# leggedrobotics/elevation_mapping_cupy

Hardware: NVIDIA B200
Metric: Mpoints/s fused + map-update frames/s (1024^2 grid, 200k-pt LiDAR frames, raycast+overlap-clear on) (higher is better)
Workload: dtype f32

## Files before the change

elevation_mapping_cupy_b200/csrc/emap_api.cu:

```cuda
#include <cmath>
#include <cstdio>
#include <cstdlib>
#include <cstring>
#include <mutex>
#include <string>
#include <vector>

#include <dlfcn.h>
#include <nvtx3/nvToolsExt.h>

#include "../../include/emap.h"
#include "emap_kernels.cuh"
#include "emap_inpaint.cuh"
#include "emap_semantic.cuh"

namespace {

thread_local std::string g_create_error;

struct StageTimer {
  cudaEvent_t ev[9];
  bool have = false;
};

// ... 292 lines not shown
      o += bytes;
    }
    CK(cudaEventRecord(h->copy_done, h->copy_stream));
    CK(cudaStreamWaitEvent(h->stream, h->copy_done, 0));
  }
  h->pend_pts.assign(dp, dp + n_sensors);
  h->pend_n.assign(n, n + n_sensors);
  h->pend_stride = row_stride; h->pend_dtype = dtype; h->pend_host = !is_device_ptr;
  h->phase = -1;
  return 0;
}

int frame_index(emap_handle* h) {
  NvtxRange nv("emap:index+error");
  const int n_sensors = (int)h->pend_pts.size();
  for (int s = 0; s < n_sensors; s++) {
    int rc = h->pend_dtype == EMAP_F32
                 ? launch_index<float>(h, h->poses[s], (const float*)h->pend_pts[s], h->pend_n[s], h->pend_stride, h->offs[s], s)
                 : launch_index<double>(h, h->poses[s], (const double*)h->pend_pts[s], h->pend_n[s], h->pend_stride, h->offs[s], s);
    if (rc) return rc;
  }
  if (h->pend_host) CK(cudaEventRecord(h->in_free[h->in_sel ^ 1], h->stream));
  if (h->zero_copy_pending) CK(cudaEventRecord(h->copy_done, h->stream));
  if (stage_mark(h, 1)) return EMAP_ERR_CUDA;
  h->phase = 1;
  return 0;
}

int frame_fuse(emap_handle* h) {
  NvtxRange nv("emap:drift+fusion");
  const float overlap_tz = h->overlap_override ? h->overlap_z_override : h->poses[0].t[2];
  if (!h->fused_drift) {
    PDL(k_drift, 1, 256, 0, h->dc, h->fs, h->pos_noise, h->ori_noise, overlap_tz, 1, h->tmap);
    LAUNCH_CHECK();
  }
  if (stage_mark(h, 2)) return EMAP_ERR_CUDA;
  if (h->fused_drift) {
    PDL((k_fuse<3, 1>), std::max(1, cdiv(h->n_points, 256)), 256, 0, h->dc, h->n_points, h->global_off, (const float4*)h->xyzv,
        (const int*)h->pidx, (const float*)h->map, h->sc, (const FrameScalars*)h->fs, h->fs, h->pos_noise, h->ori_noise, overlap_tz);
    LAUNCH_CHECK();
  } else if (h->n_points > 0) {
    if (h->attached) {
      PDL((k_fuse<1, 0>), cdiv(h->n_points, 256), 256, 0, h->dc, h->n_points, h->global_off, (const float4*)h->xyzv,
          (const int*)h->pidx, (const float*)h->map, h->sc, (const FrameScalars*)h->fs, h->fs, 0.f, 0.f, 0.f);
    } else {
      PDL((k_fuse<3, 0>), cdiv(h->n_points, 256), 256, 0, h->dc, h->n_points, h->global_off, (const float4*)h->xyzv,
          (const int*)h->pidx, (const float*)h->map, h->sc, (const FrameScalars*)h->fs, h->fs, 0.f, 0.f, 0.f);
    }
    LAUNCH_CHECK();
  }
  if (stage_mark(h, 3)) return EMAP_ERR_CUDA;
  h->phase = 2;
  return 0;
}

template <typename T>
int launch_sem_sum(emap_handle* h, const T* pts, i64 n, i64 stride, i64 off) {
  if (n <= 0) return 0;
  k_sem_sum<T><<<cdiv(n, 256), 256, 0, h->stream>>>(h->dc, h->sem, pts, n, stride, (const int*)(h->pidx + off), h->sem_fsum, h->sem_csum);
  LAUNCH_CHECK();
  return 0;
}

int frame_semantic(emap_handle* h) {
  if (h->sem.n_ch <= 0 || !h->sem_map) return 0;
  NvtxRange nv("emap:semantic");
  for (size_t s = 0; s < h->pend_pts.size(); s++) {
    int rc = h->pend_dtype == EMAP_F32
                 ? launch_sem_sum<float>(h, (const float*)h->pend_pts[s], h->pend_n[s], h->pend_stride, h->offs[s])
                 : launch_sem_sum<double>(h, (const double*)h->pend_pts[s], h->pend_n[s], h->pend_stride, h->offs[s]);
    if (rc) return rc;
  }
  if (h->pend_host) CK(cudaEventRecord(h->in_free[h->in_sel ^ 1], h->stream));
  if (h->zero_copy_pending) CK(cudaEventRecord(h->copy_done, h->stream));
  k_sem_apply<<<cdiv(h->dc.C, 256), 256, 0, h->stream>>>(h->dc, h->sem, (const u64*)h->sc.cnt_fo, h->sem_fsum, h->sem_csum, h->sem_map);
  LAUNCH_CHECK();
  return 0;
}

RayGrid ray_grid(const emap_handle* h, int align) {
  const int W = h->dc.W;
  int r0 = W, r1 = 0, c0 = W, c1 = 0;
  const double L = (double)h->dc.max_len16;
  for (const Pose& q : h->poses) {
    for (int ax = 0; ax < 2; ax++) {
      const double tc = (double)q.t[ax];
      const double e = (std::fabs(tc) + L) * (1.0 / 2048.0) + 1e-4;
      double lo = std::floor((tc - L - e) / h->dc.resolution + h->dc.half_w) - 2.0;
      double hi = std::floor((tc + L + e) / h->dc.resolution + h->dc.half_w) + 3.0;
      if (!(lo == lo) || !(hi == hi)) { lo = 0; hi = W; }
      const int a = (int)std::min(std::max(lo, 0.0), (double)W), b = (int)std::min(std::max(hi, 0.0), (double)W);
      if (ax == 0) { r0 = std::min(r0, a); r1 = std::max(r1, b); } else { c0 = std::min(c0, a); c1 = std::max(c1, b); }
    }
  }
  RayGrid g{0, 0, 0, 0, 3, 0, 0};
  if (r1 <= r0 || c1 <= c0) return g;
  c0 = (c0 / align) * align; c1 = std::min(W, ((c1 + align - 1) / align) * align);
  g.r0 = r0; g.r1 = r1; g.c0 = c0; g.c1 = c1;
  for (int ts = 2;; ts++) {
    const int al = 2 << ts;
    const int r0a = (r0 / al) * al, c0a = (c0 / al) * al;
    if ((RT << ts) >= std::max(r1 - r0a, c1 - c0a) && (4 << ts) >= h->span_cells + 1) {
      g.ts = ts; g.ta = r0a >> ts; g.tb = c0a >> ts;
      break;
    }
  }
  return g;
}

int frame_rays(emap_handle* h) {
  NvtxRange nv("emap:record+raycast");
  const bool deferred = h->attached && h->n_points > 0;
  if (deferred) {
    CK(cudaEventRecord(h->ev_fork, h->stream));
    CK(cudaStreamWaitEvent(h->side_stream, h->ev_fork, 0));
    k_fuse<2, 0><<<cdiv(h->n_points, 256), 256, 0, h->side_stream>>>(h->dc, h->n_points, h->global_off, (const float4*)h->xyzv,
                                                                       (const int*)h->pidx, (const float*)h->map, h->sc,
                                                                       (const FrameScalars*)h->fs, h->fs, 0.f, 0.f, 0.f);
    LAUNCH_CHECK();
    CK(cudaEventRecord(h->ev_join, h->side_stream));
  }
  if (h->dc.visibility) {
    const int V = (h->dc.W % 4 == 0) ? 4 : 1;
    const RayGrid box = ray_grid(h, V);
    const i64 nthreads = (i64)(box.r1 - box.r0) * ((box.c1 - box.c0) / V);
    if (nthreads > 0) {
      if (V == 4) PDL(k_record<4>, cdiv(nthreads, 256), 256, 0, h->dc, (const float*)h->map, h->sc, (const FrameScalars*)h->fs, box, h->tmap);
      else PDL(k_record<1>, cdiv(nthreads, 256), 256, 0, h->dc, (const float*)h->map, h->sc, (const FrameScalars*)h->fs, box, h->tmap);
      LAUNCH_CHECK();
    }
    if (stage_mark(h, 4)) return EMAP_ERR_CUDA;
    for (size_t s = 0; s + 1 < h->offs.size(); s++) {
      const i64 n = h->offs[s + 1] - h->offs[s];
      if (n <= 0 || h->dc.n_steps == 0) continue;
      const int grid = (int)std::min<i64>((i64)h->n_sm * h->rc_blocks_per_sm, (n + RC_THREADS / 32 - 1) / (RC_THREADS / 32));
      if (h->count_rays)
        PDL(k_raycast<true>, grid, RC_THREADS, h->rc_smem, h->dc, h->poses[s], (const Ray*)(h->rays + h->offs[s]), h->ray_ctl + RC_CTL * (int)s,
            (const float*)h->map, (const float*)h->normal, h->sc, (const float*)h->steps, h->n_tab, (const unsigned short*)h->lut, box, (const u32*)h->tmap, h->rc_lay, h->fs);
      else
        PDL(k_raycast<false>, grid, RC_THREADS, h->rc_smem, h->dc, h->poses[s], (const Ray*)(h->rays + h->offs[s]), h->ray_ctl + RC_CTL * (int)s,
            (const float*)h->map, (const float*)h->normal, h->sc, (const float*)h->steps, h->n_tab, (const unsigned short*)h->lut, box, (const u32*)h->tmap, h->rc_lay, h->fs);
      LAUNCH_CHECK();
    }
  } else if (stage_mark(h, 4)) return EMAP_ERR_CUDA;
  if (deferred) CK(cudaStreamWaitEvent(h->stream, h->ev_join, 0));
  if (stage_mark(h, 5)) return EMAP_ERR_CUDA;
  h->phase = 3;
  return 0;
}

size_t post_smem(const DevCfg& d) {
  const int HL = d.dilation + 3, HLX = (HL + 3) & ~3;
  const size_t plane = (size_t)(((PT_Y + 2 * HL) * (PT_X + 2 * HLX) + 31) & ~31);
  return sizeof(float) * (3 * plane + (size_t)(PT_Y + 6) * (PT_X + 6) + 2) + sizeof(unsigned long long) * (size_t)(PT_Y + 2 * HL + 2);
}

int make_post_tm(emap_handle* h, int which, const float* base) {
  typedef CUresult (*encode_fn)(CUtensorMap*, CUtensorMapDataType, cuuint32_t, void*, const cuuint64_t*, const cuuint64_t*,
                                const cuuint32_t*, const cuuint32_t*, CUtensorMapInterleave, CUtensorMapSwizzle,
                                CUtensorMapL2promotion, CUtensorMapFloatOOBfill);
  static encode_fn enc = nullptr;
  if (!enc) {
    void* fn = nullptr;
    cudaDriverEntryPointQueryResult qr;
    if (cudaGetDriverEntryPoint("cuTensorMapEncodeTiled", &fn, cudaEnableDefault, &qr) != cudaSuccess || !fn)
      return fail(h, EMAP_ERR_CUDA, "cuTensorMapEncodeTiled not available from the driver");
    enc = (encode_fn)fn;
  }
  memset(&h->post_tm[which], 0, sizeof(CUtensorMap));
  h->post_tm_base[which] = base;
  const int W = h->dc.W;
  const int HL = h->dc.dilation + 3, HLX = (HL + 3) & ~3;
  h->dc.post_tma = (W % 4 == 0 && W >= PT_X + 2 * HLX && W >= PT_Y + 2 * HL) ? 1 : 0;
  if (!h->dc.post_tma) return 0;
  const cuuint64_t dims[3] = {(cuuint64_t)W, (cuuint64_t)W, 7};
  const cuuint64_t strides[2] = {(cuuint64_t)W * 4, (cuuint64_t)W * W * 4};
  const cuuint32_t box[3] = {(cuuint32_t)(PT_X + 2 * HLX), (cuuint32_t)(PT_Y + 2 * HL), 1};
  const cuuint32_t es[3] = {1, 1, 1};
  const CUresult r = enc(&h->post_tm[which], CU_TENSOR_MAP_DATA_TYPE_FLOAT32, 3, (void*)base, dims, strides, box, es,
                         CU_TENSOR_MAP_INTERLEAVE_NONE, CU_TENSOR_MAP_SWIZZLE_NONE, CU_TENSOR_MAP_L2_PROMOTION_L2_128B,
                         CU_TENSOR_MAP_FLOAT_OOB_FILL_NONE);
  if (r != CUDA_SUCCESS) return fail(h, EMAP_ERR_CUDA, "cuTensorMapEncodeTiled failed");
  return 0;
}

int launch_post(emap_handle* h) {
  dim3 grid(cdiv(h->dc.W, PT_X), cdiv(h->dc.W, PT_Y));
  const size_t sm = post_smem(h->dc);
  const CUtensorMap& tm = h->post_tm[h->post_tm_base[1] == h->map ? 1 : 0];
  switch (h->dc.dilation) {
    case 1: PDL(k_post<1>, grid, 256, sm, h->dc, h->map, h->trav_input, h->normal, tm); break;
    case 2: PDL(k_post<2>, grid, 256, sm, h->dc, h->map, h->trav_input, h->normal, tm); break;
    case 3: PDL(k_post<3>, grid, 256, sm, h->dc, h->map, h->trav_input, h->normal, tm); break;
    default: PDL(k_post<0>, grid, 256, sm, h->dc, h->map, h->trav_input, h->normal, tm); break;
  }
  LAUNCH_CHECK();
  return 0;
}

int frame_finish(emap_handle* h) {
  NvtxRange nv("emap:finalize+post");
  if (h->dc.W % 4 == 0) PDL(k_finalize<4>, cdiv(h->dc.C / 4, 256), 256, 0, h->dc, h->map, h->sc, (const FrameScalars*)h->fs, h->dc.visibility, h->ray_ctl, RC_CTL * h->ray_ctl_cap, h->fused_drift ? h->fs : nullptr, h->tmap);
  else PDL(k_finalize<1>, cdiv(h->dc.C, 256), 256, 0, h->dc, h->map, h->sc, (const FrameScalars*)h->fs, h->dc.visibility, h->ray_ctl, RC_CTL * h->ray_ctl_cap, h->fused_drift ? h->fs : nullptr, h->tmap);
  LAUNCH_CHECK();
  if (stage_mark(h, 6)) return EMAP_ERR_CUDA;
  int rc = launch_post(h);
  if (rc) return rc;
  if (stage_mark(h, 7)) return EMAP_ERR_CUDA;
  h->st.have = h->timing != 0;
  h->phase = 0;
  return 0;
}

int layer_index(const char* name) {
  static const char* names[] = {"elevation", "variance", "is_valid", "traversability", "time", "upper_bound", "is_upper_bound"};
  for (int i = 0; i < 7; i++) if (!strcmp(name, names[i])) return i;
  return -1;
}

int alloc_plugin_scratch(emap_handle* h) {
  for (int i = 0; i < 4; i++) if (!h->pl[i]) CK(cudaMalloc(&h->pl[i], sizeof(float) * h->dc.C));
  return 0;
}

__global__ void k_ukey_extract(int C, const u32* __restrict__ ukv, int* __restrict__ x) {
  const int i = blockIdx.x * blockDim.x + threadIdx.x;
  if (i >= C) return;
  x[i] = (int)(ukv[i] ^ 0x80000000u);
}
__global__ void k_ukey_merge(int C, u32* __restrict__ ukv, const int* __restrict__ x) {
  const int i = blockIdx.x * blockDim.x + threadIdx.x;
  if (i >= C) return;
  ukv[i] = ((u32)x[i]) ^ 0x80000000u;
}

}

extern "C" {

const char* emap_last_error(const emap_handle* h) { return h ? h->err.c_str() : g_create_error.c_str(); }

int emap_create(const emap_config* cfg, int device, emap_handle** out) {
  if (!cfg || !out) { g_create_error = "emap_create: null argument"; return EMAP_ERR_INVALID; }
  if (cfg->abi_version != EMAP_ABI_VERSION) { g_create_error = "emap_create: abi_version mismatch"; return EMAP_ERR_INVALID; }
  if (cfg->cell_n < 8 || cfg->cell_n > 2049) {
    g_create_error = "emap_create: cell_n must be in [8, 2049]"; return EMAP_ERR_INVALID;
  }
  if (!(cfg->resolution > 0) || cfg->dilation_size < 0 || cfg->dilation_size > 8) {
    g_create_error = "emap_create: resolution > 0 and 0 <= dilation_size <= 8 required"; return EMAP_ERR_INVALID;
  }
  emap_handle* h = new emap_handle();
  h->cfg = *cfg; h->device = device;
  auto bail = [&](const char* what, cudaError_t e) {
    g_create_error = std::string(what) + ": " + cudaGetErrorString(e);
    emap_destroy(h);
    return (int)EMAP_ERR_CUDA;
  };
  cudaError_t e;
  if ((e = cudaSetDevice(device)) != cudaSuccess) return bail("cudaSetDevice", e);
  fill_devcfg(*cfg, h->dc);
  build_steps(*cfg, h->dc.max_len16, h->steps_host);
  h->dc.n_steps = (int)h->steps_host.size();
  h->dc.first_step = h->steps_host.empty() ? INFINITY : h->steps_host[0];
  const size_t C = (size_t)h->dc.C;
  if ((e = cudaStreamCreateWithFlags(&h->own_stream, cudaStreamNonBlocking)) != cudaSuccess) return bail("stream", e);
  h->stream = h->own_stream;
  if ((e = cudaStreamCreateWithFlags(&h->copy_stream, cudaStreamNonBlocking)) != cudaSuccess) return bail("stream", e);
  for (int b = 0; b < 2; b++) {
    if ((e = cudaEventCreateWithFlags(&h->in_free[b], cudaEventDisableTiming)) != cudaSuccess) return bail("event", e);
    if ((e = cudaEventRecord(h->in_free[b], h->stream)) != cudaSuccess) return bail("event", e);
  }
  if ((e = cudaEventCreateWithFlags(&h->copy_done, cudaEventDisableTiming)) != cudaSuccess) return bail("event", e);
  if ((e = cudaStreamCreateWithFlags(&h->side_stream, cudaStreamNonBlocking)) != cudaSuccess) return bail("stream", e);
  if ((e = cudaEventCreateWithFlags(&h->ev_fork, cudaEventDisableTiming)) != cudaSuccess) return bail("event", e);
  if ((e = cudaEventCreateWithFlags(&h->ev_join, cudaEventDisableTiming)) != cudaSuccess) return bail("event", e);
  if ((e = cudaEventCreateWithFlags(&h->ev_order, cudaEventDisableTiming)) != cudaSuccess) return bail("event", e);
  for (int k = 0; k < 9; k++) if ((e = cudaEventCreate(&h->st.ev[k])) != cudaSuccess) return bail("event", e);
#define ALLOC(p, bytes) if ((e = cudaMalloc(&(p), (bytes))) != cudaSuccess) return bail("cudaMalloc", e)
#define TRY(call) if ((e = (call)) != cudaSuccess) return bail(#call, e)
  ALLOC(h->map, sizeof(float) * 7 * C);
  ALLOC(h->map_alt, sizeof(float) * 7 * C);
  ALLOC(h->normal, sizeof(float) * 3 * C);
  ALLOC(h->trav_input, sizeof(float) * C);
  ALLOC(h->u32_block, sizeof(u32) * 5 * C);
  ALLOC(h->i64_block, sizeof(i64) * 3 * C);
  ALLOC(h->sc.last, sizeof(u64) * C);
  ALLOC(h->sc.rec, sizeof(uint2) * C);
  ALLOC(h->sc.thr, sizeof(float) * C);
  ALLOC(h->sc.ukv, sizeof(u32) * C);
  ALLOC(h->dirty, C + 16);
  ALLOC(h->ukey_x, sizeof(int) * C);
  ALLOC(h->fs, sizeof(FrameScalars));
  ALLOC(h->lut, sizeof(unsigned short) * 65536);
  ALLOC(h->tmap, sizeof(u32) * RT * RT);
  ALLOC(h->step_cnt, sizeof(unsigned short) * (0x7c00 + 8));
  ALLOC(h->d_export, sizeof(float) * C);
  h->d_export_floats = C;
  h->n_tab = (int)(((h->steps_host.size() + RC_STRIDE - 1) / RC_STRIDE) * RC_STRIDE + 64) & ~1;
  ALLOC(h->steps, sizeof(float) * h->n_tab);
#undef ALLOC
  h->sc.cnt_ai = (u64*)h->u32_block; h->sc.cnt_fo = (u64*)(h->u32_block + 2 * C); h->sc.n_ray = h->u32_block + 4 * C;
  h->sc.SH = h->i64_block; h->sc.SV = h->i64_block + C; h->sc.DV = h->i64_block + 2 * C;
  h->sc.dirty = h->dirty;
  TRY(cudaMemsetAsync(h->u32_block, 0, sizeof(u32) * 5 * C, h->stream));
  TRY(cudaMemsetAsync(h->i64_block, 0, sizeof(i64) * 3 * C, h->stream));
  TRY(cudaMemsetAsync(h->sc.last, 0, sizeof(u64) * C, h->stream));
  TRY(cudaMemsetAsync(h->sc.rec, 0, sizeof(uint2) * C, h->stream));
// ... 826 lines not shown
```

elevation_mapping_cupy_b200/csrc/emap_kernels.cuh:

```cuda
#pragma once
#include <cuda.h>
#include "emap_device.cuh"

struct CellScratch {
  u64* cnt_ai;
  u64* cnt_fo;
  u32* n_ray;
  i64* SH;
  i64* SV;
  i64* DV;
  u64* last;
  float* thr;
  uint2* rec;
  u32* ukv;
  unsigned char* dirty;
  i64 mc_off;
};

#define RT 64
struct RayGrid { int r0, r1, c0, c1, ts, ta, tb; };

__device__ __forceinline__ void red_add(u32* p, u32 v, i64 mc) {
  if (mc) asm volatile("multimem.red.relaxed.sys.global.add.u32 [%0], %1;" ::"l"((char*)p + mc), "r"(v) : "memory");
  else atomicAdd(p, v);
// ... 558 lines not shown
  }
}

__device__ __forceinline__ void finalize_cell(const DevCfg& c, float* __restrict__ map, const CellScratch& s, const int i,
                                              const int rr, const int cc, const int applied, const float shift,
                                              const float hmin, const float hmax, const int rays_ran) {
  const size_t C = (size_t)c.C;
  const u64 fo = s.cnt_fo[i], ca = s.cnt_ai[i];
  u32 nr = 0, kv = UKEY_NONE;
  i64 dv_fix = 0;
  if (rays_ran) { nr = s.n_ray[i]; kv = s.ukv[i]; dv_fix = s.DV[i]; }
  const u64 last_key = s.last[i];
  const i64 sh_fix = s.SH[i], sv_fix = s.SV[i];
  const u32 cf = (u32)fo, no = (u32)(fo >> 32);
  const float h0 = map[i], v0 = map[C + i], va0 = map[2 * C + i], ti0 = map[4 * C + i], up0 = map[5 * C + i], iu0 = map[6 * C + i];
  float h = h0, v = v0, valid = va0, time = ti0, upper = up0, isup = iu0;
  if (applied) h = __fadd_rn(h, shift);
  v = add_n_times(v, c.c_out, no);
  if (cf > 0) {
    valid = 1.f; time = 0.f; isup = 0.f;
    upper = __uint_as_float((u32)(last_key & 0xffffffffull));
  }
  if (rays_ran) {
    const u32 key0 = (isup < 0.5f) ? UKEY_NONE : fkey(upper);
    if (nr > 0) {
      valid = __fadd_rn(valid, (float)unfix32(dv_fix));
      v = add_n_times(v, c.c_out, nr);
    }
    const u32 ukey = min(key0, kv);
    if (ukey != key0) { upper = funkey(ukey); isup = 1.f; }
  }
  const float valid_in = valid;
  if (cf > 0) {
    const double cnt = (double)cf;
    const float mean_v = (float)(unfix32(sv_fix) / cnt);
    if ((double)mean_v > c.max_variance) { h = 0.f; v = c.init_var; valid = 0.f; }
    else { h = (float)(unfix32(sh_fix) / cnt); v = mean_v; valid = 1.f; }
  }
  if (valid_in < 0.5f) { h = 0.f; v = c.init_var; valid = 0.f; }
  if (c.overlap && rr >= c.cell_min && rr < c.cell_max && cc >= c.cell_min && cc < c.cell_max) {
    if (h < hmin || h > hmax) { h = 0.f; v = c.init_var; valid = 0.f; }
    if (upper < hmin || upper > hmax) { upper = 0.f; isup = 0.f; }
  }
  if (applied || h != h0) map[i] = h;
  if (v != v0) map[C + i] = v;
  if (valid != va0) map[2 * C + i] = valid;
  if (time != ti0) map[4 * C + i] = time;
  if (upper != up0) map[5 * C + i] = upper;
  if (isup != iu0) map[6 * C + i] = isup;
  if (cf) { s.SH[i] = 0; s.SV[i] = 0; s.last[i] = 0; }
  if (fo) s.cnt_fo[i] = 0;
  if (nr) { s.DV[i] = 0; s.n_ray[i] = 0; }
  if (ca) s.cnt_ai[i] = 0;
  if (kv != UKEY_NONE) s.ukv[i] = UKEY_NONE;
}

#ifndef FIN_MINB
#define FIN_MINB 4
#endif
template <int V>
__global__ void __launch_bounds__(256, FIN_MINB)
k_finalize(const DevCfg c, float* __restrict__ map, const CellScratch s, const FrameScalars* __restrict__ fs,
           const int rays_ran, int* __restrict__ ray_ctl, const int n_ctl, FrameScalars* fs_reset, u32* __restrict__ tmap) {
  __shared__ int s_list[8][32 * V];
  pdl_trigger(); pdl_wait();
  if (blockIdx.x == 0) for (int k = threadIdx.x; k < n_ctl; k += blockDim.x) ray_ctl[k] = 0;
  if (fs_reset && blockIdx.x == 1 % gridDim.x) {
    for (int k = threadIdx.x; k < RT * RT; k += blockDim.x) tmap[k] = 0u;
    if (threadIdx.x == 0) { fs_reset->E = 0; fs_reset->ecnt = 0; fs_reset->nvalid = 0; }
  }
  const int lane = threadIdx.x & 31, wid = threadIdx.x >> 5;
  const int i0 = (blockIdx.x * blockDim.x + threadIdx.x) * V;
  const size_t C = (size_t)c.C;
  const int applied = fs->applied;
  const float shift = fs->shift;
  u32 full = 0;
  int r = 0, col0 = 0;
  if (i0 < c.C) {
    r = i0 / c.W; col0 = i0 - r * c.W;
    if (s.dirty) {
      if (V == 4) {
        const u32 d = *reinterpret_cast<const u32*>(s.dirty + i0);
        if (d) {
          *reinterpret_cast<u32*>(s.dirty + i0) = 0u;
          full = ((d & 0xffu) ? 1u : 0u) | ((d & 0xff00u) ? 2u : 0u) | ((d & 0xff0000u) ? 4u : 0u) | ((d & 0xff000000u) ? 8u : 0u);
        }
      } else {
        for (int j = 0; j < V; j++) if (s.dirty[i0 + j]) { full |= 1u << j; s.dirty[i0 + j] = 0; }
      }
    } else {
      u64 ca[V]; u32 kv[V];
      ldv64<V>(s.cnt_ai + i0, ca); ldv<V>(s.ukv + i0, kv);
      for (int j = 0; j < V; j++) if (ca[j] != 0ull || kv[j] != UKEY_NONE) full |= 1u << j;
    }
    if (c.overlap && r >= c.cell_min && r < c.cell_max)
      for (int j = 0; j < V; j++) if (col0 + j >= c.cell_min && col0 + j < c.cell_max) full |= 1u << j;
    if (full != (1u << V) - 1u) {
      float h0[V], v0[V], va0[V], h4[V], v4[V], va4[V];
      ldv<V>(map + i0, h0); ldv<V>(map + C + i0, v0); ldv<V>(map + 2 * C + i0, va0);
#pragma unroll
      for (int j = 0; j < V; j++) {
        const bool inval = va0[j] < 0.5f;
        h4[j] = inval ? 0.f : (applied ? __fadd_rn(h0[j], shift) : h0[j]);
        v4[j] = inval ? c.init_var : v0[j];
        va4[j] = inval ? 0.f : va0[j];
      }
      if (full == 0) {
        if (applied || diffv<V>(h4, h0)) stv<V>(map + i0, h4);
        if (diffv<V>(v4, v0)) stv<V>(map + C + i0, v4);
        if (diffv<V>(va4, va0)) stv<V>(map + 2 * C + i0, va4);
      } else {
#pragma unroll
        for (int j = 0; j < V; j++) {
          if ((full >> j) & 1u) continue;
          if (applied || h4[j] != h0[j]) map[i0 + j] = h4[j];
          if (v4[j] != v0[j]) map[C + i0 + j] = v4[j];
          if (va4[j] != va0[j]) map[2 * C + i0 + j] = va4[j];
        }
      }
    }
  }
  const int nfull = __popc(full);
  int incl = nfull;
#pragma unroll
  for (int d = 1; d < 32; d <<= 1) { const int o = __shfl_up_sync(0xffffffffu, incl, d); if (lane >= d) incl += o; }
  const int total = __shfl_sync(0xffffffffu, incl, 31);
  if (total == 0) return;
  int pos = incl - nfull;
  for (int j = 0; j < V; j++) if ((full >> j) & 1u) s_list[wid][pos++] = i0 + j;
  __syncwarp();
  const float hmin = __fsub_rn(fs->overlap_tz, c.overlap_z_f), hmax = __fadd_rn(fs->overlap_tz, c.overlap_z_f);
  for (int e = lane; e < total; e += 32) {
    const int i = s_list[wid][e];
    const int rr = i / c.W;
    finalize_cell(c, map, s, i, rr, i - rr * c.W, applied, shift, hmin, hmax, rays_ran);
  }
}

#define PT_X 32
#ifndef PT_Y
#define PT_Y 16
#endif

__device__ __forceinline__ void ffma2(float2& acc, const float2 w, const float t) {
  u64 a, ww, tt;
  asm("mov.b64 %0, {%1, %2};" : "=l"(a) : "f"(acc.x), "f"(acc.y));
  asm("mov.b64 %0, {%1, %2};" : "=l"(ww) : "f"(w.x), "f"(w.y));
  asm("mov.b64 %0, {%1, %1};" : "=l"(tt) : "f"(t));
  asm("fma.rn.f32x2 %0, %1, %2, %0;" : "+l"(a) : "l"(ww), "l"(tt));
  asm("mov.b64 {%0, %1}, %2;" : "=f"(acc.x), "=f"(acc.y) : "l"(a));
}

template <int KT>
__global__ void __launch_bounds__(256)
k_post(const DevCfg c, float* __restrict__ map, float* __restrict__ trav_input, float* __restrict__ normal,
       const __grid_constant__ CUtensorMap tm) {
  extern __shared__ __align__(128) float smem[];
  pdl_trigger(); pdl_wait();
  const int W = c.W, C = c.C;
  const int K = KT ? KT : c.dilation;
  const int HL = K + 3;
  const int HLX = (HL + 3) & ~3;
  const int A = PT_Y + 2 * HL, B = PT_X + 2 * HLX;
  constexpr int DA = PT_Y + 6, DB = PT_X + 6;
  const int PS = (A * B + 31) & ~31;
  float* s_up = smem;
  float* s_mask = s_up + PS;
  float* s_iu = s_mask + PS;
  float* s_dil = s_iu + PS;
  unsigned long long* s_rowsel = reinterpret_cast<unsigned long long*>(s_dil + DA * DB + ((DA * DB) & 1));
  unsigned long long* s_bar = s_rowsel + A;
  const float* up = map + 5 * C; const float* valid = map + 2 * C; const float* isup = map + 6 * C;
  const int r0 = blockIdx.y * PT_Y, c0 = blockIdx.x * PT_X;
  const int tid = threadIdx.x, tx = tid & 31, ty = tid >> 5;
  const bool bulk = c.post_tma != 0;
  if (bulk) {
    const u32 sbar = (u32)__cvta_generic_to_shared(s_bar);
    if (tid == 0) {
      asm volatile("mbarrier.init.shared::cta.b64 [%0], 1;" ::"r"(sbar));
      asm volatile("fence.mbarrier_init.release.cluster;" ::: "memory");
      asm volatile("mbarrier.arrive.expect_tx.shared::cta.b64 _, [%0], %1;" ::"r"(sbar), "r"(3 * A * B * 4) : "memory");
#pragma unroll
      for (int pl = 0; pl < 3; pl++) {
        const u32 dst = (u32)__cvta_generic_to_shared(pl == 0 ? s_up : pl == 1 ? s_mask : s_iu);
        asm volatile("cp.async.bulk.tensor.3d.shared::cluster.global.mbarrier::complete_tx::bytes [%0], [%1, {%2, %3, %4}], [%5];"
                     ::"r"(dst), "l"(&tm), "r"(c0 - HLX), "r"(r0 - HL), "r"(pl == 0 ? 5 : pl == 1 ? 2 : 6), "r"(sbar) : "memory");
      }
    }
    __syncthreads();
    u32 ok = 0;
    while (!ok)
      asm volatile("{ .reg .pred p; mbarrier.try_wait.parity.shared::cta.b64 p, [%1], %2; selp.u32 %0, 1, 0, p; }"
                   : "=r"(ok) : "r"(sbar), "r"(0) : "memory");
  }
  int any_sel = 0;
  for (int a = ty; a < A; a += 8) {
    const int r = r0 - HL + a;
    u32 bits[2];
#pragma unroll
    for (int ch = 0; ch < 2; ch++) {
      const int b = tx + 32 * ch;
      const int cc = c0 - HLX + b;
      float m = 0.f;
      const bool in_stage = b < B;
      if (bulk) {
        if (in_stage) { m = __fadd_rn(s_mask[a * B + b], s_iu[a * B + b]); s_mask[a * B + b] = m; }
      } else {
        float u = 0.f;
        if (in_stage && r >= 0 && r < W && cc >= 0 && cc < W) {
          const int gi = r * W + cc;
          u = __ldg(up + gi);
          m = __fadd_rn(__ldg(valid + gi), __ldg(isup + gi));
        }
        if (in_stage) { s_up[a * B + b] = u; s_mask[a * B + b] = m; }
      }
      const bool sel = in_stage && r > 0 && r < W - 1 && cc > 0 && cc < W - 1 && m > 0.5f;
      bits[ch] = __ballot_sync(0xffffffffu, sel);
    }
    if (tx == 0) s_rowsel[a] = ((unsigned long long)bits[1] << 32) | bits[0];
    any_sel |= (bits[0] | bits[1]) != 0;
  }
  any_sel = __syncthreads_or(any_sel);
  for (int e = tid; e < DA * DB; e += 256) {
    const int a = e / DB, b = e - a * DB;
    const int r = r0 - 3 + a, cc = c0 - 3 + b;
    float out = 0.f;
    if (r >= 0 && r < W && cc >= 0 && cc < W) {
      if (cc >= K - 1 && cc <= W - K) {
        const int sa = a + K, sb = b + HLX - 3;
        out = s_up[sa * B + sb];
        if (any_sel && s_mask[sa * B + sb] < 0.5f) {
          if (KT) {
            constexpr int KK = KT ? KT : 1;
            const u32 wmask = (1u << (2 * KK + 1)) - 1u;
            u32 term[2 * KK + 1], any = 0;
#pragma unroll
            for (int i = 0; i <= 2 * KK; i++) {
              term[i] = ((u32)(s_rowsel[sa + i - KK] >> (sb - KK)) & wmask) << i;
              any |= term[i];
            }
            if (any) {
              const int sp = __ffs(any) - 1;
              int iw = 2 * KK;
#pragma unroll
              for (int i = 2 * KK - 1; i >= 0; i--) if ((term[i] >> sp) & 1u) iw = i;
              out = s_up[(sa + iw - KK) * B + sb + (sp - iw - KK)];
            }
          } else {
            const u64 wmask = (1ull << (2 * K + 1)) - 1ull;
            u64 any = 0;
            for (int dy = -K; dy <= K; dy++)
              any |= ((s_rowsel[sa + dy] >> (sb - K)) & wmask) << (dy + K);
            if (any) {
              const int sp = __ffsll((long long)any) - 1;
              int dyw = K;
              for (int dy = K; dy >= -K; dy--) {
                const int dx = sp - (dy + K) - K;
                if (dx >= -K && dx <= K && ((s_rowsel[sa + dy] >> (sb + dx)) & 1ull)) dyw = dy;
              }
              out = s_up[(sa + dyw) * B + sb + (sp - (dyw + K) - K)];
            }
          }
        }
      }
    }
    s_dil[e] = out;
  }
  if (K >= 2 && (c0 - 3 < K - 1 || c0 + PT_X + 3 > W - K)) {
    __syncthreads();
    const int lane = tid & 31, warp = tid >> 5, side = 2 * K + 1;
    const int la = max(c0 - 3, 0), nl = max(0, min(c0 - 3 + DB - 1, K - 2) - la + 1);
    const int ra = max(max(c0 - 3, W - K + 1), K - 1), nr = max(0, min(c0 - 3 + DB - 1, W - 1) - ra + 1);
    const int nc = nl + nr;
    for (int e2 = warp; e2 < DA * nc; e2 += 8) {
      const int a = e2 / nc, j = e2 - a * nc;
      const int r = r0 - 3 + a, cc = j < nl ? la + j : ra + (j - nl);
      const int e = a * DB + (cc - (c0 - 3));
      if (r < 0 || r >= W) continue;
      const int i = r * W + cc;
      float out = up[i];
      if (__fadd_rn(valid[i], isup[i]) < 0.5f) {
        u32 best = 0xffffffffu;
        for (int cand = lane; cand < side * side; cand += 32) {
          const int dy = cand / side - K, dx = cand - (dy + K) * side - K;
          int rr = r + dy, c2 = cc + dx;
          if (c2 < 0) { c2 += W; rr -= 1; } else if (c2 >= W) { c2 -= W; rr += 1; }
          if (rr <= 0 || rr >= W - 1 || c2 <= 0 || c2 >= W - 1) continue;
          const int idx = rr * W + c2;
          if (__fadd_rn(valid[idx], isup[idx]) > 0.5f) best = min(best, (u32)((dx + dy + 2 * K) << 8 | (dy + K)));
        }
        best = __reduce_min_sync(0xffffffffu, best);
        if (best != 0xffffffffu) {
          const int dy = (int)(best & 255u) - K, dx = (int)(best >> 8) - 2 * K - dy;
          int rr = r + dy, c2 = cc + dx;
          if (c2 < 0) { c2 += W; rr -= 1; } else if (c2 >= W) { c2 -= W; rr += 1; }
          out = up[rr * W + c2];
        }
      }
      if (lane == 0) s_dil[e] = out;
    }
  }
  __syncthreads();
#pragma unroll
  for (int half = 0; half < PT_Y / 8; half++) {
    const int a = ty + half * 8, b = tx;
    const int r = r0 + a, cc = c0 + b;
    if (r >= W || cc >= W) continue;
    const int gi = r * W + cc;
    const float* d = s_dil + (a + 3) * DB + (b + 3);
    const float h = d[0];
    trav_input[gi] = h;
    if (r >= 3 && r <= W - 4 && cc >= 3 && cc <= W - 4) {
      float acc = 0.f;
#pragma unroll
      for (int l = 0; l < 3; l++) {
        const int dil = l + 1;
        float t[9];
#pragma unroll
        for (int p = 0; p < 3; p++)
#pragma unroll
          for (int qq = 0; qq < 3; qq++) t[p * 3 + qq] = d[(p - 1) * dil * DB + (qq - 1) * dil];
#pragma unroll
        for (int cp = 0; cp < 2; cp++) {
          float2 s2 = make_float2(0.f, 0.f);
#pragma unroll
          for (int j = 0; j < 9; j++) ffma2(s2, c.wp[l][cp][j], t[j]);
          acc = __fmaf_rn(c.wout[l * 4 + 2 * cp], fabsf(s2.x), acc);
          acc = __fmaf_rn(c.wout[l * 4 + 2 * cp + 1], fabsf(s2.y), acc);
        }
      }
      map[3 * C + gi] = expf(-acc);
    }
    float n0 = 0.f, n1 = 0.f, n2 = 0.f;
    if (__ldg(valid + gi) > 0.5f && r >= 1 && r <= W - 3 && cc >= 1 && cc <= W - 3) {
      const float dzdx = __fsub_rn(d[1], h), dzdy = __fsub_rn(d[DB], h);
      const float nx = __fdiv_rn(-dzdy, c.res_f), ny = __fdiv_rn(-dzdx, c.res_f);
      const float nn = __fsqrt_rn(__fadd_rn(__fmaf_rn(nx, nx, __fmul_rn(ny, ny)), 1.0f));
      n0 = __fdiv_rn(nx, nn); n1 = __fdiv_rn(ny, nn); n2 = __fdiv_rn(1.0f, nn);
    }
    normal[gi] = n0; normal[C + gi] = n1; normal[2 * C + gi] = n2;
  }
}

__global__ void __launch_bounds__(256)
k_normal(const DevCfg c, const float* __restrict__ dil, const float* __restrict__ valid, float* __restrict__ normal) {
  const int i = blockIdx.x * blockDim.x + threadIdx.x;
  if (i >= c.C) return;
  const int W = c.W, r = i / W, cc = i - r * W;
  float n0 = 0.f, n1 = 0.f, n2 = 0.f;
  if (valid[i] > 0.5f && r >= 1 && r <= W - 3 && cc >= 1 && cc <= W - 3) {
    const float h = dil[i];
    const float dzdx = __fsub_rn(dil[i + 1], h), dzdy = __fsub_rn(dil[i + W], h);
    const float nx = __fdiv_rn(-dzdy, c.res_f), ny = __fdiv_rn(-dzdx, c.res_f);
    const float nn = __fsqrt_rn(__fadd_rn(__fmaf_rn(nx, nx, __fmul_rn(ny, ny)), 1.0f));
    n0 = __fdiv_rn(nx, nn); n1 = __fdiv_rn(ny, nn); n2 = __fdiv_rn(1.0f, nn);
  }
  normal[i] = n0; normal[c.C + i] = n1; normal[2 * c.C + i] = n2;
}

__global__ void __launch_bounds__(256)
k_shift(const DevCfg c, const float* __restrict__ src, float* __restrict__ dst, int sx, int sy, double dz) {
  const int i = blockIdx.x * blockDim.x + threadIdx.x;
  if (i >= c.C) return;
  const int W = c.W, r = i / W, cc = i - r * W;
  const size_t C = (size_t)c.C;
  const bool pad = (sx > 0 && r < sx) || (sx < 0 && r >= W + sx) || (sy > 0 && cc < sy) || (sy < 0 && cc >= W + sy);
  float v[7];
  if (pad) {
#pragma unroll
    for (int l = 0; l < 7; l++) v[l] = (l == L_V) ? c.init_var : 0.f;
  } else {
    int rs = r - sx, cs = cc - sy;
    rs = ((rs % W) + W) % W; cs = ((cs % W) + W) % W;
    const size_t si = (size_t)rs * W + cs;
#pragma unroll
    for (int l = 0; l < 7; l++) v[l] = __ldg(src + l * C + si);
  }
  v[L_H] = (float)((double)v[L_H] + dz); v[L_UPPER] = (float)((double)v[L_UPPER] + dz);
#pragma unroll
  for (int l = 0; l < 7; l++) dst[l * C + i] = v[l];
}
__global__ void __launch_bounds__(256) k_shift_z(const DevCfg c, float* __restrict__ map, double dz) {
  const int i = blockIdx.x * blockDim.x + threadIdx.x;
  if (i >= c.C) return;
  map[i] = (float)((double)map[i] + dz);
  map[5 * c.C + i] = (float)((double)map[5 * c.C + i] + dz);
}
__global__ void __launch_bounds__(256) k_clear(const DevCfg c, float* __restrict__ map) {
  const int i = blockIdx.x * blockDim.x + threadIdx.x;
  if (i >= c.C) return;
  for (int l = 0; l < 7; l++) map[(size_t)l * c.C + i] = (l == L_V) ? c.init_var : 0.f;
}
__global__ void __launch_bounds__(256) k_init(const DevCfg c, float* __restrict__ map) {
  const int i = blockIdx.x * blockDim.x + threadIdx.x;
  if (i >= c.C) return;
  for (int l = 0; l < 7; l++) map[(size_t)l * c.C + i] = (l == L_V) ? c.init_var : (l == L_TRAV ? 1.f : 0.f);
}
__global__ void __launch_bounds__(256) k_update_variance(const DevCfg c, float* __restrict__ map) {
  const int i = blockIdx.x * blockDim.x + threadIdx.x;
  if (i >= c.C) return;
  map[c.C + i] = __fadd_rn(map[c.C + i], __fmul_rn(c.time_var_f, map[2 * c.C + i]));
}
__global__ void __launch_bounds__(256) k_update_time(const DevCfg c, float* __restrict__ map) {
  const int i = blockIdx.x * blockDim.x + threadIdx.x;
  if (i >= c.C) return;
  map[4 * c.C + i] = __fadd_rn(map[4 * c.C + i], c.time_int_f);
}

__global__ void __launch_bounds__(256)
k_init_dilate(const DevCfg c, const float* __restrict__ src_h, const float* __restrict__ src_valid, float* __restrict__ map,
              int k, int last) {
  const int i = blockIdx.x * blockDim.x + threadIdx.x;
  if (i >= c.C) return;
  const int W = c.W, C = c.C;
  float h = src_h[i], valid = src_valid[i];
  if (valid < 0.5f) {
    float distance = 100.f, near_value = 0.f;
    for (int dy = -k; dy <= k; dy++)
      for (int dx = -k; dx <= k; dx++) {
        const int idx = i + W * dy + dx;
        if (idx < 0 || idx >= C) continue;
        const int ix = idx / W, iy = idx - ix * W;
        if (ix <= 0 || ix >= W - 1 || iy <= 0 || iy >= W - 1) continue;
        if (src_valid[idx] > 0.5f && (float)(dx + dy) < distance) { distance = (float)(dx + dy); near_value = src_h[idx]; }
      }
    if (distance < 100.f) { h = near_value; valid = 1.0f; }
  }
  map[i] = h; map[2 * C + i] = valid;
  if (last && valid > 0.5f) { map[5 * C + i] = h; map[6 * C + i] = 0.f; }
}

__device__ __forceinline__ float export_value(const DevCfg& c, const float* __restrict__ map, const float* __restrict__ normal,
                                              int o, int kind, float center_z, int only_above, const float* __restrict__ plane,
                                              int flags) {
  const int Wo = c.W - 2;
  const int orow = o / Wo, ocol = o - orow * Wo;
  const int r = Wo - 1 - orow + 1, cc = Wo - 1 - ocol + 1;
  const int i = r * c.W + cc, C = c.C;
  const float nanv = __int_as_float(0x7fc00000);
  const float valid = map[2 * C + i], isup = map[6 * C + i], upper = map[5 * C + i];
  float v;
  switch (kind) {
    case 0: v = (valid > 0.5f) ? __fadd_rn(map[i], center_z) : nanv; break;
    case 1: v = map[C + i]; break;
    case 2: {
      const bool in33 = r >= 3 && r <= c.W - 4 && cc >= 3 && cc <= c.W - 4;
      v = (in33 && __fadd_rn(valid, isup) > 0.5f) ? map[3 * C + i] : nanv; break; }
    case 3: v = map[4 * C + i]; break;
    case 4: case 5: {
      const bool ok = only_above ? ((upper > 0.f && isup > 0.5f) || valid > 0.5f) : (valid > 0.5f || isup > 0.5f);
      v = ok ? (kind == 4 ? __fadd_rn(upper, center_z) : isup) : nanv; break; }
    case 9: {
      v = plane[i];
      if ((flags & 1) && !(valid > 0.5f)) v = nanv;
      if (flags & 2) v = __fadd_rn(v, center_z);
      break; }
    default: v = normal[(size_t)(kind - 6) * C + i]; break;
  }
  return v;
}

__global__ void __launch_bounds__(256)
k_export(const DevCfg c, const float* __restrict__ map, const float* __restrict__ normal, float* __restrict__ out,
         int kind, float center_z, int only_above, const float* __restrict__ plane, int flags) {
  const int Wo = c.W - 2;
  const int o = blockIdx.x * blockDim.x + threadIdx.x;
  if (o >= Wo * Wo) return;
  out[o] = export_value(c, map, normal, o, kind, center_z, only_above, plane, flags);
}

#define EXPORT_MAX_LAYERS 24
struct ExportList { int n; int kind[EXPORT_MAX_LAYERS]; int flags[EXPORT_MAX_LAYERS]; const float* plane[EXPORT_MAX_LAYERS]; };
__global__ void __launch_bounds__(256)
k_export_multi(const DevCfg c, const float* __restrict__ map, const float* __restrict__ normal, float* __restrict__ out,
               const ExportList L, float center_z, int only_above) {
  const int Wo = c.W - 2;
  const int o = blockIdx.x * blockDim.x + threadIdx.x;
  const int l = blockIdx.y;
  if (o >= Wo * Wo) return;
  out[(size_t)l * Wo * Wo + o] = export_value(c, map, normal, o, L.kind[l], center_z, only_above, L.plane[l], L.flags[l]);
}

__global__ void __launch_bounds__(256)
k_min_filter_iter(const DevCfg c, int k, const float* __restrict__ mask0, const float* __restrict__ in_h,
                  const float* __restrict__ in_m, float* __restrict__ out_h, float* __restrict__ out_m,
                  int* __restrict__ unfilled, int it, int is_max) {
  if (it > 0 && unfilled[it - 1] == 0) { if (blockIdx.x == 0 && threadIdx.x == 0) unfilled[it] = 0; return; }
  const int i = blockIdx.x * blockDim.x + threadIdx.x;
// ... 117 lines not shown
```

Measured before the change: 1484.

## Dilate in place in staged tile using row bitmasks and drop dilation buffer

The post-processing kernel no longer fills a separate dilated-height shared buffer. It overwrites the staged height plane in place, and only for candidate cells, which are found by OR-ing neighbouring row-selection bitmasks and intersecting them with per-row 'need' masks. It also reads the valid mask from shared memory instead of global memory, and adds a minimum-blocks hint to __launch_bounds__. The aim is less shared-memory footprint, so more blocks fit per SM, and less per-cell work, at the cost of more complex bitmask logic and register pressure from the occupancy hint.

New measurement: 1493 (median of 6 runs). No clear change (+0.6%).

```diff
diff --git a/elevation_mapping_cupy_b200/csrc/emap_api.cu b/elevation_mapping_cupy_b200/csrc/emap_api.cu
--- a/elevation_mapping_cupy_b200/csrc/emap_api.cu
+++ b/elevation_mapping_cupy_b200/csrc/emap_api.cu
@@ -468,7 +468,7 @@
 size_t post_smem(const DevCfg& d) {
   const int HL = d.dilation + 3, HLX = (HL + 3) & ~3;
   const size_t plane = (size_t)(((PT_Y + 2 * HL) * (PT_X + 2 * HLX) + 31) & ~31);
-  return sizeof(float) * (3 * plane + (size_t)(PT_Y + 6) * (PT_X + 6) + 2) + sizeof(unsigned long long) * (size_t)(PT_Y + 2 * HL + 2);
+  return sizeof(float) * 3 * plane + sizeof(unsigned long long) * (size_t)(2 * (PT_Y + 2 * HL) + 1);
 }
 
 int make_post_tm(emap_handle* h, int which, const float* base) {
diff --git a/elevation_mapping_cupy_b200/csrc/emap_kernels.cuh b/elevation_mapping_cupy_b200/csrc/emap_kernels.cuh
--- a/elevation_mapping_cupy_b200/csrc/emap_kernels.cuh
+++ b/elevation_mapping_cupy_b200/csrc/emap_kernels.cuh
@@ -734,7 +734,7 @@
 }
 
 template <int KT>
-__global__ void __launch_bounds__(256)
+__global__ void __launch_bounds__(256, KT ? 8 : 6)
 k_post(const DevCfg c, float* __restrict__ map, float* __restrict__ trav_input, float* __restrict__ normal,
        const __grid_constant__ CUtensorMap tm) {
   extern __shared__ __align__(128) float smem[];
@@ -745,13 +745,14 @@
   const int HLX = (HL + 3) & ~3;
   const int A = PT_Y + 2 * HL, B = PT_X + 2 * HLX;
   constexpr int DA = PT_Y + 6, DB = PT_X + 6;
+  const int X = HLX - 3;
   const int PS = (A * B + 31) & ~31;
   float* s_up = smem;
-  float* s_mask = s_up + PS;
-  float* s_iu = s_mask + PS;
-  float* s_dil = s_iu + PS;
-  unsigned long long* s_rowsel = reinterpret_cast<unsigned long long*>(s_dil + DA * DB + ((DA * DB) & 1));
-  unsigned long long* s_bar = s_rowsel + A;
+  float* s_valid = s_up + PS;
+  float* s_iu = s_valid + PS;
+  u64* s_rowsel = reinterpret_cast<u64*>(s_iu + PS);
+  u64* s_rowneed = s_rowsel + A;
+  u64* s_bar = s_rowneed + A;
   const float* up = map + 5 * C; const float* valid = map + 2 * C; const float* isup = map + 6 * C;
   const int r0 = blockIdx.y * PT_Y, c0 = blockIdx.x * PT_X;
   const int tid = threadIdx.x, tx = tid & 31, ty = tid >> 5;
@@ -764,21 +765,31 @@
       asm volatile("mbarrier.arrive.expect_tx.shared::cta.b64 _, [%0], %1;" ::"r"(sbar), "r"(3 * A * B * 4) : "memory");
 #pragma unroll
       for (int pl = 0; pl < 3; pl++) {
-        const u32 dst = (u32)__cvta_generic_to_shared(pl == 0 ? s_up : pl == 1 ? s_mask : s_iu);
+        const u32 dst = (u32)__cvta_generic_to_shared(pl == 0 ? s_up : pl == 1 ? s_valid : s_iu);
         asm volatile("cp.async.bulk.tensor.3d.shared::cluster.global.mbarrier::complete_tx::bytes [%0], [%1, {%2, %3, %4}], [%5];"
                      ::"r"(dst), "l"(&tm), "r"(c0 - HLX), "r"(r0 - HL), "r"(pl == 0 ? 5 : pl == 1 ? 2 : 6), "r"(sbar) : "memory");
       }
     }
+  }
+  u64 colsel, dcols;
+  {
+    const int s0 = c0 - HLX + tx, s1 = s0 + 32, d0 = c0 - 3 + tx, d1 = d0 + 32;
+    colsel = ((u64)__ballot_sync(0xffffffffu, tx + 32 < B && s1 > 0 && s1 < W - 1) << 32) |
+             __ballot_sync(0xffffffffu, s0 > 0 && s0 < W - 1);
+    dcols = ((u64)__ballot_sync(0xffffffffu, tx + 32 < DB && d1 >= K - 1 && d1 <= W - K) << 32) |
+            __ballot_sync(0xffffffffu, d0 >= K - 1 && d0 <= W - K);
+  }
+  if (bulk) {
+    const u32 sbar = (u32)__cvta_generic_to_shared(s_bar);
     __syncthreads();
     u32 ok = 0;
     while (!ok)
       asm volatile("{ .reg .pred p; mbarrier.try_wait.parity.shared::cta.b64 p, [%1], %2; selp.u32 %0, 1, 0, p; }"
                    : "=r"(ok) : "r"(sbar), "r"(0) : "memory");
   }
-  int any_sel = 0;
   for (int a = ty; a < A; a += 8) {
     const int r = r0 - HL + a;
-    u32 bits[2];
+    u32 sel[2], need[2];
 #pragma unroll
     for (int ch = 0; ch < 2; ch++) {
       const int b = tx + 32 * ch;
@@ -786,67 +797,75 @@
       float m = 0.f;
       const bool in_stage = b < B;
       if (bulk) {
-        if (in_stage) { m = __fadd_rn(s_mask[a * B + b], s_iu[a * B + b]); s_mask[a * B + b] = m; }
+        if (in_stage) m = __fadd_rn(s_valid[a * B + b], s_iu[a * B + b]);
       } else {
-        float u = 0.f;
+        float u = 0.f, v = 0.f;
         if (in_stage && r >= 0 && r < W && cc >= 0 && cc < W) {
           const int gi = r * W + cc;
-          u = __ldg(up + gi);
-          m = __fadd_rn(__ldg(valid + gi), __ldg(isup + gi));
-        }
-        if (in_stage) { s_up[a * B + b] = u; s_mask[a * B + b] = m; }
-      }
-      const bool sel = in_stage && r > 0 && r < W - 1 && cc > 0 && cc < W - 1 && m > 0.5f;
-      bits[ch] = __ballot_sync(0xffffffffu, sel);
-    }
-    if (tx == 0) s_rowsel[a] = ((unsigned long long)bits[1] << 32) | bits[0];
-    any_sel |= (bits[0] | bits[1]) != 0;
-  }
-  any_sel = __syncthreads_or(any_sel);
-  for (int e = tid; e < DA * DB; e += 256) {
-    const int a = e / DB, b = e - a * DB;
-    const int r = r0 - 3 + a, cc = c0 - 3 + b;
-    float out = 0.f;
-    if (r >= 0 && r < W && cc >= 0 && cc < W) {
-      if (cc >= K - 1 && cc <= W - K) {
-        const int sa = a + K, sb = b + HLX - 3;
-        out = s_up[sa * B + sb];
-        if (any_sel && s_mask[sa * B + sb] < 0.5f) {
-          if (KT) {
-            constexpr int KK = KT ? KT : 1;
-            const u32 wmask = (1u << (2 * KK + 1)) - 1u;
-            u32 term[2 * KK + 1], any = 0;
-#pragma unroll
-            for (int i = 0; i <= 2 * KK; i++) {
-              term[i] = ((u32)(s_rowsel[sa + i - KK] >> (sb - KK)) & wmask) << i;
-              any |= term[i];
-            }
-            if (any) {
-              const int sp = __ffs(any) - 1;
-              int iw = 2 * KK;
-#pragma unroll
-              for (int i = 2 * KK - 1; i >= 0; i--) if ((term[i] >> sp) & 1u) iw = i;
-              out = s_up[(sa + iw - KK) * B + sb + (sp - iw - KK)];
-            }
-          } else {
-            const u64 wmask = (1ull << (2 * K + 1)) - 1ull;
-            u64 any = 0;
-            for (int dy = -K; dy <= K; dy++)
-              any |= ((s_rowsel[sa + dy] >> (sb - K)) & wmask) << (dy + K);
-            if (any) {
-              const int sp = __ffsll((long long)any) - 1;
-              int dyw = K;
-              for (int dy = K; dy >= -K; dy--) {
-                const int dx = sp - (dy + K) - K;
-                if (dx >= -K && dx <= K && ((s_rowsel[sa + dy] >> (sb + dx)) & 1ull)) dyw = dy;
-              }
-              out = s_up[(sa + dyw) * B + sb + (sp - (dyw + K) - K)];
-            }
-          }
-        }
-      }
-    }
-    s_dil[e] = out;
+          u = __ldg(up + gi); v = __ldg(valid + gi);
+          m = __fadd_rn(v, __ldg(isup + gi));
+        }
+        if (in_stage) { s_up[a * B + b] = u; s_valid[a * B + b] = v; }
+      }
+      sel[ch] = __ballot_sync(0xffffffffu, m > 0.5f);
+      need[ch] = __ballot_sync(0xffffffffu, m < 0.5f);
+    }
+    if (tx == 0) {
+      s_rowsel[a] = (r > 0 && r < W - 1) ? ((((u64)sel[1] << 32) | sel[0]) & colsel) : 0ull;
+      s_rowneed[a] = ((u64)need[1] << 32) | need[0];
+    }
+  }
+  __syncthreads();
+  for (int a = ty; a < DA; a += 8) {
+    const int r = r0 - 3 + a;
+    if (r < 0 || r >= W) continue;
+    const int sa = a + K;
+    constexpr int KK = KT ? KT : 1;
+    u64 w[2 * KK + 1], v = 0;
+    if (KT) {
+#pragma unroll
+      for (int i = 0; i <= 2 * KK; i++) { w[i] = s_rowsel[sa + i - KK]; v |= w[i]; }
+    } else {
+      for (int dy = -K; dy <= K; dy++) v |= s_rowsel[sa + dy];
+    }
+    u64 spread = v;
+    for (int dx = 1; dx <= K; dx++) spread |= (v >> dx) | (v << dx);
+    const u64 cand = ((s_rowneed[sa] & spread) >> X) & dcols;
+    if (!cand) continue;
+#pragma unroll
+    for (int ch = 0; ch < 2; ch++) {
+      const int b = tx + 32 * ch;
+      if (!((cand >> b) & 1ull)) continue;
+      const int sb = b + X;
+      float out;
+      if (KT) {
+        const u32 wmask = (1u << (2 * KK + 1)) - 1u;
+        u32 term[2 * KK + 1], any = 0;
+#pragma unroll
+        for (int i = 0; i <= 2 * KK; i++) {
+          term[i] = ((u32)(w[i] >> (sb - KK)) & wmask) << i;
+          any |= term[i];
+        }
+        const int sp = __ffs(any) - 1;
+        int iw = 2 * KK;
+#pragma unroll
+        for (int i = 2 * KK - 1; i >= 0; i--) if ((term[i] >> sp) & 1u) iw = i;
+        out = s_up[(sa + iw - KK) * B + sb + (sp - iw - KK)];
+      } else {
+        const u64 wmask = (1ull << (2 * K + 1)) - 1ull;
+        u64 any = 0;
+        for (int dy = -K; dy <= K; dy++)
+          any |= ((s_rowsel[sa + dy] >> (sb - K)) & wmask) << (dy + K);
+        const int sp = __ffsll((long long)any) - 1;
+        int dyw = K;
+        for (int dy = K; dy >= -K; dy--) {
+          const int dx = sp - (dy + K) - K;
+          if (dx >= -K && dx <= K && ((s_rowsel[sa + dy] >> (sb + dx)) & 1ull)) dyw = dy;
+        }
+        out = s_up[(sa + dyw) * B + sb + (sp - (dyw + K) - K)];
+      }
+      s_up[sa * B + sb] = out;
+    }
   }
   if (K >= 2 && (c0 - 3 < K - 1 || c0 + PT_X + 3 > W - K)) {
     __syncthreads();
@@ -857,7 +876,6 @@
     for (int e2 = warp; e2 < DA * nc; e2 += 8) {
       const int a = e2 / nc, j = e2 - a * nc;
       const int r = r0 - 3 + a, cc = j < nl ? la + j : ra + (j - nl);
-      const int e = a * DB + (cc - (c0 - 3));
       if (r < 0 || r >= W) continue;
       const int i = r * W + cc;
       float out = up[i];
@@ -879,7 +897,7 @@
           out = up[rr * W + c2];
         }
       }
-      if (lane == 0) s_dil[e] = out;
+      if (lane == 0) s_up[(a + K) * B + (cc - (c0 - 3)) + X] = out;
     }
   }
   __syncthreads();
@@ -889,7 +907,8 @@
     const int r = r0 + a, cc = c0 + b;
     if (r >= W || cc >= W) continue;
     const int gi = r * W + cc;
-    const float* d = s_dil + (a + 3) * DB + (b + 3);
+    const int si = (a + HL) * B + (b + HLX);
+    const float* d = s_up + si;
     const float h = d[0];
     trav_input[gi] = h;
     if (r >= 3 && r <= W - 4 && cc >= 3 && cc <= W - 4) {
@@ -901,7 +920,7 @@
 #pragma unroll
         for (int p = 0; p < 3; p++)
 #pragma unroll
-          for (int qq = 0; qq < 3; qq++) t[p * 3 + qq] = d[(p - 1) * dil * DB + (qq - 1) * dil];
+          for (int qq = 0; qq < 3; qq++) t[p * 3 + qq] = d[(p - 1) * dil * B + (qq - 1) * dil];
 #pragma unroll
         for (int cp = 0; cp < 2; cp++) {
           float2 s2 = make_float2(0.f, 0.f);
@@ -914,8 +933,8 @@
       map[3 * C + gi] = expf(-acc);
     }
     float n0 = 0.f, n1 = 0.f, n2 = 0.f;
-    if (__ldg(valid + gi) > 0.5f && r >= 1 && r <= W - 3 && cc >= 1 && cc <= W - 3) {
-      const float dzdx = __fsub_rn(d[1], h), dzdy = __fsub_rn(d[DB], h);
+    if (s_valid[si] > 0.5f && r >= 1 && r <= W - 3 && cc >= 1 && cc <= W - 3) {
+      const float dzdx = __fsub_rn(d[1], h), dzdy = __fsub_rn(d[B], h);
       const float nx = __fdiv_rn(-dzdy, c.res_f), ny = __fdiv_rn(-dzdx, c.res_f);
       const float nn = __fsqrt_rn(__fadd_rn(__fmaf_rn(nx, nx, __fmul_rn(ny, ny)), 1.0f));
       n0 = __fdiv_rn(nx, nn); n1 = __fdiv_rn(ny, nn); n2 = __fdiv_rn(1.0f, nn);
```
